# lukehollis/three-mlagents

Hardware: AMD Instinct MI355X
Metric: env_steps_per_sec (higher is better)
Workload: dtype f32; 1 GPU; gridworld, 4096 envs/GPU, full PPO iterations: n_steps=1024, MLP pi/vf 64x64 tanh, n_epochs=10, batch_size=131072/GPU (32 minibatches/epoch), lr=3e-4, gamma=0.99, gae_lambda=0.95, clip=0.2, ent=0.01, vf=0.5, max_grad_norm=0.5; envs_per_gpu=4096, n_steps=1024, batch_size=131072, n_epochs=10, hidden=64, parallelism=single GPU

## Files before the change

include/tma.h:

```cpp
#ifndef TMA_H
#define TMA_H

#include <stdint.h>

#ifdef __cplusplus
extern "C" {
#endif

#define TMA_VERSION 211

enum { TMA_OK = 0, TMA_ERR_INVALID = 1, TMA_ERR_UNKNOWN_TASK = 2, TMA_ERR_HIP = 3 };

enum { TMA_TASK_BASIC = 0, TMA_TASK_GRIDWORLD = 1, TMA_TASK_BALL3D = 2, TMA_TASK_PUSH = 3, TMA_TASK_CRAWLER = 4, TMA_TASK_WALLJUMP = 5, TMA_TASK_BICYCLE = 6, TMA_TASK_BRICKBREAK = 7, TMA_TASK_GLIDER = 8,
       TMA_TASK_ANT = 9,
       TMA_NUM_TASKS = 10 };

enum { TMA_ACT_I32 = 0, TMA_ACT_I64 = 1, TMA_ACT_F32 = 2 };

#define TMA_EP_STRIDE (1u << 20)

int tma_version(void);
const char *tma_last_error(void);

int tma_task_id(const char *name, int *task_out);
// ... 92 lines not shown
                           const tma_ppo_hparams *hp, float *grad, void *workspace, void *stream);
int tma_ppo_epoch_prepare(const tma_rollout *rb, const tma_minibatch *epoch, int64_t batch_size, const tma_policy_dims *d, void *workspace,
                          void *stream);
int tma_ppo_epoch_adv_sums(void *workspace, const tma_policy_dims *d, int64_t batch_size, int64_t total, double *sums, int direction,
                           void *stream);
int tma_ppo_adam_step(float *params, float *grad, float *exp_avg, float *exp_avg_sq, const tma_policy_dims *d, int64_t step, double lr,
                      double beta1, double beta2, double eps, double max_grad_norm, double grad_scale, void *workspace, void *stream);
int tma_ppo_adam_step_local(float *params, float *grad, float *exp_avg, float *exp_avg_sq, const tma_policy_dims *d, int64_t step, double lr,
                            double beta1, double beta2, double eps, double max_grad_norm, void *workspace, void *stream, int64_t last_count);
int tma_ppo_train_epoch_local(float *params, const tma_policy_dims *d, const tma_rollout *rb, uint32_t perm_seed, uint32_t perm_epoch,
                              int64_t batch_size, const tma_ppo_hparams *hp, float *grad, float *exp_avg, float *exp_avg_sq, int64_t first_step,
                              double lr, double beta1, double beta2, double eps, double max_grad_norm, void *workspace, void *stream);
int tma_ppo_train_epochs_local(float *params, const tma_policy_dims *d, const tma_rollout *rb, uint32_t perm_seed, uint32_t perm_epoch0, int n_epochs,
                               int64_t batch_size, const tma_ppo_hparams *hp, float *grad, float *exp_avg, float *exp_avg_sq, int64_t first_step,
                               double lr, double beta1, double beta2, double eps, double max_grad_norm, void *workspace, void *stream);
typedef int (*tma_allreduce_fn)(void *ctx, float *buffer, int64_t count);
int tma_ppo_train_epoch_dp(float *params, const tma_policy_dims *d, const tma_rollout *rb, uint32_t perm_seed, uint32_t perm_epoch,
                           int64_t batch_size, int64_t prepared_batch, int stats_world, const tma_ppo_hparams *hp, float *grad, float *exp_avg,
                           float *exp_avg_sq, int64_t first_step, double lr, double beta1, double beta2, double eps, double max_grad_norm,
                           double grad_scale, tma_allreduce_fn allreduce, void *ctx, void *workspace, void *stream);
typedef struct tma_comm tma_comm;
int tma_comm_available(void);
int tma_comm_unique_id(unsigned char *id_out128);
int tma_comm_create(const unsigned char *id128, int world, int rank, int device, tma_comm **out);
int tma_comm_destroy(tma_comm *comm);
int tma_comm_bind_stream(tma_comm *comm, void *stream);
int tma_comm_allreduce(tma_comm *comm, void *buffer, int64_t count, int dtype, void *stream);
int tma_comm_allreduce_cb(void *ctx, float *buffer, int64_t count);
int tma_comm_timing(tma_comm *comm, int samples);
int tma_comm_pop_timing(tma_comm *comm, float *us_out, int capacity, int *n_out, int64_t *calls_out);
// ... 65 lines not shown
```

three-mlagents_amd/_lib.py:

```python
from __future__ import annotations

import ctypes as C
import os

_HERE = os.path.dirname(os.path.abspath(__file__))
SO_PATH = os.environ.get("TMA_LIB_PATH") or os.path.join(_HERE, "csrc", "libtma_hip.so")

TMA_OK, TMA_ERR_INVALID, TMA_ERR_UNKNOWN_TASK, TMA_ERR_HIP = 0, 1, 2, 3
ACT_I32, ACT_I64, ACT_F32 = 0, 1, 2
EP_STRIDE = 1 << 20
EV_SCRATCH_DOUBLES = 1536

_vp, _i32, _i64, _u32, _f64 = C.c_void_p, C.c_int, C.c_int64, C.c_uint32, C.c_double



class PolicyDims(C.Structure):
    _fields_ = [("obs_dim", _i32), ("hidden", _i32), ("act_dim", _i32), ("continuous", _i32), ("mfma_dtype", _i32), ("device", _i32)]


class Rollout(C.Structure):
    _fields_ = [("obs", _vp), ("actions", _vp), ("log_probs", _vp), ("advantages", _vp), ("returns", _vp), ("T", _i32), ("N", _i64),
                ("packed", _vp)]

# ... 50 lines not shown
    "tma_policy_sync": (_i32, [_vp, _pd, _vp]),
    "tma_policy_act": (_i32, [_vp, _pd, _vp, _i64, _u32, _u32, _u32, _i32, _vp, _vp, _vp, _vp]),
    "tma_policy_act_bootstrap": (_i32, [_vp, _pd, _vp, _i64, _u32, _u32, _u32, _vp, _vp, _vp, _vp, _vp, _f64, _vp, _vp]),
    "tma_policy_evaluate_actions": (_i32, [_vp, _pd, _vp, _vp, _i64, _vp, _vp, _vp, _vp]),
    "tma_policy_values": (_i32, [_vp, _pd, _vp, _i64, _vp, _vp]),
    "tma_policy_bootstrap": (_i32, [_vp, _pd, _vp, _vp, _i64, _f64, _vp, _vp]),
    "tma_ppo_workspace_bytes": (_i64, [_pd]),
    "tma_ppo_packed_floats": (_i64, [_pd, _i32, _i64]),
    "tma_ppo_pack_samples": (_i32, [C.POINTER(Rollout), _pd, _vp, _vp]),
    "tma_ppo_minibatch_grad": (_i32, [_vp, _pd, C.POINTER(Rollout), C.POINTER(Minibatch), C.POINTER(PPOHParams), _vp, _vp, _vp]),
    "tma_debug_time_grad_kernel": (_i32, [_i32]),
    "tma_debug_poison_lds": (_i32, [_u32, _vp]),
    "tma_debug_last_grad_kernel_us": (_i32, [C.POINTER(C.c_float)]),
    "tma_debug_last_dispatch": (_i32, [C.POINTER(_i32), C.POINTER(_i32), C.POINTER(_i32)]),
    "tma_debug_last_rollout_waves": (_i32, []),
    "tma_ppo_epoch_prepare": (_i32, [C.POINTER(Rollout), C.POINTER(Minibatch), _i64, _pd, _vp, _vp]),
    "tma_ppo_epoch_adv_sums": (_i32, [_vp, _pd, _i64, _i64, _vp, _i32, _vp]),
    "tma_ppo_adam_step": (_i32, [_vp, _vp, _vp, _vp, _pd, _i64, _f64, _f64, _f64, _f64, _f64, _f64, _vp, _vp]),
    "tma_ppo_adam_step_local": (_i32, [_vp, _vp, _vp, _vp, _pd, _i64, _f64, _f64, _f64, _f64, _f64, _vp, _vp, _i64]),
    "tma_ppo_permutation": (_i32, [_u32, _u32, _i64, _vp]),
    "tma_ppo_persist_fallbacks": (_i32, [_vp, C.POINTER(_i64), _vp]),
    "tma_ppo_train_epoch_local": (_i32, [_vp, _pd, C.POINTER(Rollout), _u32, _u32, _i64, C.POINTER(PPOHParams), _vp, _vp, _vp, _i64, _f64, _f64, _f64, _f64,
                                         _f64, _vp, _vp]),
    "tma_ppo_train_epochs_local": (_i32, [_vp, _pd, C.POINTER(Rollout), _u32, _u32, _i32, _i64, C.POINTER(PPOHParams), _vp, _vp, _vp, _i64, _f64, _f64, _f64, _f64,
                                          _f64, _vp, _vp]),
    "tma_ppo_train_epoch_dp": (_i32, [_vp, _pd, C.POINTER(Rollout), _u32, _u32, _i64, _i64, _i32, C.POINTER(PPOHParams), _vp, _vp, _vp, _i64, _f64, _f64, _f64,
                                      _f64, _f64, _f64, None, _vp, _vp, _vp]),
    "tma_ppo_pop_stats": (_i32, [_vp, C.POINTER(_f64), _vp]),
    "tma_ppo_stats_staging_bytes": (_i64, []),
    "tma_ppo_stats_enqueue": (_i32, [_vp, _vp, _vp]),
# ... 77 lines not shown
```

three-mlagents_amd/csrc/tma_h64.hip:

```cpp
#include "tma_h64_tile.h"

#include <cstdlib>

namespace tma {


template <int KT, int NT>
__device__ __forceinline__ void bwd_weight_acc(const float *xin, int ldx, int K, const float *dz, int ldz, int N, f32x4 (&accW)[KT][NT],
                                               float (&accb)[NT], int lane) {
    (void)K, (void)N;
    const int r16 = lane & 15, g = lane >> 4;
    float bf[NT][4];
#pragma unroll
    for (int nt = 0; nt < NT; nt++) {
        const int col = nt * 16 + r16;
#pragma unroll
        for (int s = 0; s < 4; s++) bf[nt][s] = dz[(4 * s + g) * ldz + col];
        accb[nt] += (bf[nt][0] + bf[nt][1]) + (bf[nt][2] + bf[nt][3]);
    }
#pragma unroll
    for (int kt = 0; kt < KT; kt++) {
        const int krow = kt * 16 + r16;
        float a[4];
#pragma unroll
// ... 358 lines not shown
        for (int i = 0; i < NO; i++) {
            const int y = o_tid + i * o_thr, x = y < w2_off ? y : y + 4096;
            if (y < n_other) {
                const float gv = (go[i] * f.scale) * coef;
                const float pnew = adam_update_h64(po[i], gv, mo[i], vo[i], f.beta1, f.beta2, inv_bc2, f.eps, f.lr_step);
                image_store_h64(wimg, L.D, n_out, x, pnew);
                if (keep) f.p_nxt[base + x] = pnew, f.m_nxt[base + x] = mo[i], f.v_nxt[base + x] = vo[i];
            }
        }
    }
}

template <bool IS_PI, int DT, bool DIRECT = false, int AT = 0>
__device__ __forceinline__ void grad_h64t_body(const float *__restrict__ params, const PLayout &L, const Rollout &rb, const Minibatch &mb,
                                               const HParams &hp, const double *__restrict__ adv_part, int n_part, float *__restrict__ slab,
                                               double *__restrict__ stat_slot, float *smem, int n_blocks_net, int block_net, const AdamFold &fold) {
#ifdef TMA_H64_TICKS
    const unsigned long long kern_t0 = __builtin_amdgcn_s_memtime();
#endif
    __shared__ float adv_ms[2];
    const int lane = threadIdx.x & 63, wave = threadIdx.x >> 6, wpb = blockDim.x >> 6;
    const int r16 = lane & 15, g = lane >> 4;
    (void)0;
    const int D = DT > 0 ? DT : L.D, A = AT > 0 ? AT : L.A;
    constexpr int KS1C = DT > 0 ? (DT + 3) / 4 : 4;
    const int KS1 = (D + 3) >> 2;
    float *wimg = smem;
    float *slotA = smem + IMG_FLOATS + wave * T_PER_WAVE, *slotB = slotA + 16 * LDT, *dz3t = slotB + 16 * LDT, *Xt = dz3t + 256;
    const float invB = 1.0f / (float)mb.count;
    const int NOUT = IS_PI ? A : 1;
    const int64_t n_tiles = (mb.count + 15) >> 4;
// ... 107 lines not shown
        for (int q = 0; q < 5; q++) red[wave * 5 + q] = stv[q];
    if constexpr (DIRECT) {
        flush_all_t<IS_PI, KS1C, 4>(smem, wave, lane, acc, L, D, NOUT, slab);
    } else {
        flush_all_t<IS_PI, KS1C>(smem, wave, lane, acc, L, D, NOUT, slab);
    }
#ifdef TMA_H64_TICKS
    if (tick_on && lane == 0) g_h64_ticks[IS_PI ? 0 : 1][13] += __builtin_amdgcn_s_memtime() - loop_t1;
#endif
    if (threadIdx.x < 5) {
        double s = 0.0;
        for (int w = 0; w < wpb; w++) s += red[w * 5 + threadIdx.x];
        const int q = IS_PI ? (threadIdx.x == 0 ? 0 : threadIdx.x + 1) : (threadIdx.x == 0 ? 1 : -1);
        if (q >= 0) stat_slot[q] += s;
    }
}

template <int DT, int VER, int AT = 0>
__global__ __launch_bounds__(512, 2) void ppo_grad_h64_kernel(const float *__restrict__ params, PLayout L, Rollout rb, Minibatch mb, HParams hp,
                                                              const double *__restrict__ adv_part, int n_part, float *__restrict__ slabs,
                                                              double *__restrict__ stat_slots, AdamFold fold) {
    extern __shared__ __attribute__((aligned(16))) float smem[];
    const int n_pairs = gridDim.x >> 1, pair = (int)blockIdx.x % n_pairs;
    const bool pi_block = (int)blockIdx.x < n_pairs;
    float *slab = slabs + (int64_t)pair * L.P;
    double *slot = stat_slots + (int64_t)pair * 8;
    if constexpr (VER == 1) {
        if (pi_block) grad_h64_body<true, DT>(params, L, rb, mb, hp, adv_part, n_part, slab, slot, smem, n_pairs, pair);
        else grad_h64_body<false, DT>(params, L, rb, mb, hp, adv_part, n_part, slab, slot, smem, n_pairs, pair);
    } else {
        if (pi_block) grad_h64t_body<true, DT, false, AT>(params, L, rb, mb, hp, adv_part, n_part, slab, slot, smem, n_pairs, pair, fold);
        else grad_h64t_body<false, DT>(params, L, rb, mb, hp, adv_part, n_part, slab, slot, smem, n_pairs, pair, fold);
    }
}

template <int DT>
__global__ __launch_bounds__(256, 1) void ppo_grad_h64_small_kernel(const float *__restrict__ params, PLayout L, Rollout rb, Minibatch mb, HParams hp,
                                                                    const double *__restrict__ adv_part, int n_part, float *__restrict__ slabs,
                                                                    double *__restrict__ stat_slots, AdamFold fold) {
    extern __shared__ __attribute__((aligned(16))) float smem[];
    const int pair = blockIdx.x >> 1, n_pairs = gridDim.x >> 1;
    float *slab = slabs + (int64_t)pair * L.P;
    double *slot = stat_slots + (int64_t)pair * 8;
    if ((blockIdx.x & 1) == 0) grad_h64t_body<true, DT, true>(params, L, rb, mb, hp, adv_part, n_part, slab, slot, smem, n_pairs, pair, fold);
    else grad_h64t_body<false, DT, true>(params, L, rb, mb, hp, adv_part, n_part, slab, slot, smem, n_pairs, pair, fold);
}

}

using namespace tma;

static int grad_h64_smem_bytes(const PLayout &L, int wpb, int ver) {
    const int ldx = ((L.D + 3) & ~3) + 2, ld = L.H + 2;
    const int per_wave = ver == 1 ? 16 * (ldx + 2 * ld + 34) + 16 * 8 : T_PER_WAVE;
    const int tile = (IMG_FLOATS + wpb * per_wave) * 4;
    const int flush = wpb * (L.H * L.H + L.H) * 4;
    return tile > flush ? tile : flush;
}

int tma_launch_grad_h64(const float *params, const PLayout &L, const Rollout &R, const Minibatch &M, const HParams &hpar, const double *adv_part,
                        int n_part, float *slabs, double *slots, int *n_slabs_out, hipStream_t s, const AdamFold *foldp) {
    AdamFold fold{};
    if (foldp) fold = *foldp;
    static const int ver = getenv("TMA_H64_V1") ? 1 : 2;
    if (ver == 1 && foldp && foldp->grad) return TMA_ERR_INVALID;
    static const int stagger = getenv("TMA_H64_STAGGER") ? atoi(getenv("TMA_H64_STAGGER")) : 0;
    static const bool runtime_a = getenv("TMA_H64_RUNTIME_A") != nullptr;
    HParams hps = hpar;
    hps.debug = stagger;
    const int64_t tiles = ceil_div(M.count, 16);
    if (ver == 2 && tiles <= H64_BLOCKS) {
        const int64_t blocks = ceil_div(tiles, 4);
        const int smem = (IMG_FLOATS + 4 * T_PER_WAVE) * 4;
        auto launch_small = [&](auto k) -> int {
            TMA_HIP(hipFuncSetAttribute(reinterpret_cast<const void *>(k), hipFuncAttributeMaxDynamicSharedMemorySize, smem));
            k<<<dim3((unsigned)(2 * blocks)), dim3(256), smem, s>>>(params, L, R, M, hps, adv_part, n_part, slabs, slots, fold);
            return TMA_OK;
        };
        const int rc = L.D == 4 ? launch_small(ppo_grad_h64_small_kernel<4>) : (L.D == 6 ? launch_small(ppo_grad_h64_small_kernel<6>) : launch_small(ppo_grad_h64_small_kernel<0>));
        if (rc) return rc;
        TMA_LAUNCH_CHECK();
        *n_slabs_out = (int)blocks;
        return TMA_OK;
    }
    const int wpb4 = 8, smem4 = grad_h64_smem_bytes(L, wpb4, ver);
    int64_t blocks4 = ceil_div(tiles, wpb4);
    if (blocks4 > H64_BLOCKS) blocks4 = H64_BLOCKS;
    auto launch = [&](auto k) -> int {
        if (smem4 > 64 * 1024) TMA_HIP(hipFuncSetAttribute(reinterpret_cast<const void *>(k), hipFuncAttributeMaxDynamicSharedMemorySize, smem4));
        k<<<dim3((unsigned)(2 * blocks4)), dim3(64 * wpb4), smem4, s>>>(params, L, R, M, hps, adv_part, n_part, slabs, slots, fold);
        return TMA_OK;
    };
    int rc;
    if (ver == 1) rc = L.D == 4 ? launch(ppo_grad_h64_kernel<4, 1>) : (L.D == 6 ? launch(ppo_grad_h64_kernel<6, 1>) : launch(ppo_grad_h64_kernel<0, 1>));
    else if (L.D == 4 && L.A == 5 && !runtime_a) rc = launch(ppo_grad_h64_kernel<4, 2, 5>);
    else rc = L.D == 4 ? launch(ppo_grad_h64_kernel<4, 2>) : (L.D == 6 ? launch(ppo_grad_h64_kernel<6, 2>) : launch(ppo_grad_h64_kernel<0, 2>));
    if (rc) return rc;
    TMA_LAUNCH_CHECK();
    *n_slabs_out = (int)blocks4;
    return TMA_OK;
}

#ifdef TMA_H64_TICKS
extern "C" int tma_debug_h64_ticks(unsigned long long *out32, int reset) {
    TMA_HIP(hipDeviceSynchronize());
    if (out32) TMA_HIP(hipMemcpyFromSymbol(out32, HIP_SYMBOL(g_h64_ticks), sizeof(unsigned long long) * 32));
    if (reset) {
        unsigned long long z[32] = {};
        TMA_HIP(hipMemcpyToSymbol(HIP_SYMBOL(g_h64_ticks), z, sizeof(z)));
    }
    return TMA_OK;
}
#endif
```

three-mlagents_amd/csrc/tma_policy.hip:

```cpp
#include "tma_h64_tile.h"
#include "tma_p2p.h"

#include <cstring>
#include <cmath>
#include <cstdio>
#include <cstdlib>
#include <type_traits>
#include <vector>

namespace tma {


__device__ __forceinline__ void build_image_elem(float *params, const PLayout &L, int img, int e, int W1t, int b1, int W2t, int b2, int W3t, int b3,
                                                 int n_out) {
    const int D = L.D, H = 64;
    float v = 0.0f;
    if (e < IMG_W2F) {
        const int x = e - IMG_W1, k = x >> 6, r16 = (x >> 2) & 15, j = x & 3;
        v = k < D ? params[W1t + k * H + 16 * j + r16] : 0.0f;
    } else if (e < IMG_W3F) {
        const int x = e - IMG_W2F, k = x >> 6, r16 = (x >> 2) & 15, j = x & 3;
        v = params[W2t + k * H + 16 * j + r16];
    } else if (e < IMG_W3B) {
        const int x = e - IMG_W3F, k = x >> 4, col = x & 15;
// ... 219 lines not shown
                            if (entropy_out != nullptr) entropy_out[row] = entsum;
                        }
                        continue;
                    }
                    const float vrow = gfirst_quad(vacc[0][r]);
                    if (r16 == r && row < n) {
                        logp_out[row] = lpsum;
                        values_out[row] = vrow;
                    }
                }
            }
        }
    }
}

constexpr int ADV_BLOCKS = 128;
__global__ __launch_bounds__(256) void adv_partial_kernel(const float *__restrict__ adv, Minibatch mb, int T, int64_t N, double *partials,
                                                          int32_t *__restrict__ offs_out, int64_t batch = 0) {
    __shared__ double s1[4], s2[4];
    if (gridDim.y > 1 || batch > 0) {
        const int64_t k = blockIdx.y, s0 = k * batch;
        const int64_t cnt = (s0 + batch <= mb.count) ? batch : mb.count - s0;
        mb.start += s0, mb.count = cnt;
        partials += 2 * k * gridDim.x;
        if (offs_out) offs_out += s0;
    }
    int nb = (int)((mb.count + 1023) / 1024);
    if (nb > (int)gridDim.x) nb = gridDim.x;
    if ((int)blockIdx.x >= nb) return;
    const int64_t per = (mb.count + nb - 1) / nb;
    const int64_t j0 = (int64_t)blockIdx.x * per, j1 = (j0 + per < mb.count) ? j0 + per : mb.count;
    double a = 0.0, b = 0.0;
    for (int64_t j = j0 + threadIdx.x; j < j1; j += 256) {
        const int64_t off = sample_offset(mb, mb.start + j, T, N);
        if (offs_out) offs_out[j] = (int32_t)off;
        const double x = (double)adv[off];
        a += x;
        b += x * x;
    }
    for (int o = 32; o > 0; o >>= 1) {
        a += __shfl_down(a, o, 64);
        b += __shfl_down(b, o, 64);
    }
    if ((threadIdx.x & 63) == 0) s1[threadIdx.x >> 6] = a, s2[threadIdx.x >> 6] = b;
    __syncthreads();
    if (threadIdx.x == 0) {
        partials[2 * blockIdx.x] = (s1[0] + s1[1]) + (s1[2] + s1[3]);
        partials[2 * blockIdx.x + 1] = (s2[0] + s2[1]) + (s2[2] + s2[3]);
    }
}
__global__ void adv_final_kernel(const double *partials, int n_part, int64_t count, float *ws_adv) {
    double a = 0.0, b = 0.0;
    for (int k = threadIdx.x; k < n_part; k += 64) a += partials[2 * k], b += partials[2 * k + 1];
    for (int o = 32; o > 0; o >>= 1) {
        a += __shfl_down(a, o, 64);
        b += __shfl_down(b, o, 64);
    }
    if (threadIdx.x == 0) {
        const double n = (double)count, mean = a / n;
        double var = n > 1.0 ? (b - n * mean * mean) / (n - 1.0) : 0.0;
        if (var < 0.0) var = 0.0;
        ws_adv[0] = (float)mean;
        ws_adv[1] = (float)sqrt(var);
    }
// ... 2052 lines not shown
    if (n < 1) return fail(TMA_ERR_INVALID, "tma_policy_values: n must be >= 1");
    return launch_fwd<1>(params, d, obs, n, 0, 0, 0, 1, nullptr, values_out, nullptr, nullptr, 0.0f, nullptr, (hipStream_t)stream);
}

int tma_policy_bootstrap(const float *params, const tma_policy_dims *d, const float *terminal_obs, const uint8_t *truncated, int64_t n, double gamma,
                         float *rewards_inout, void *stream) {
    g_disp_fwd = TMA_DISPATCH_NONE;
    int rc = enter(d);
    if (rc) return rc;
    if (!params || !terminal_obs || !truncated || !rewards_inout) return fail(TMA_ERR_INVALID, "tma_policy_bootstrap: null buffer");
    if (n < 1) return fail(TMA_ERR_INVALID, "tma_policy_bootstrap: n must be >= 1");
    return launch_fwd<2>(params, d, terminal_obs, n, 0, 0, 0, 1, nullptr, nullptr, nullptr, truncated, (float)gamma, rewards_inout, (hipStream_t)stream);
}

static int minibatch_grad_impl(const float *params, const tma_policy_dims *d, const tma_rollout *rb, const tma_minibatch *mbi, const tma_ppo_hparams *hp,
                               float *grad, void *workspace, void *stream, const AdamFold *fold, int overwrite, const PeerPush *push = nullptr) {
    g_disp_grad = TMA_DISPATCH_NONE;
    int rc = enter(d);
    if (rc) return rc;
    if (!params || !rb || !mbi || !hp || !grad || !workspace) return fail(TMA_ERR_INVALID, "tma_ppo_minibatch_grad: null argument");
    if (!rb->obs || !rb->actions || !rb->log_probs || !rb->advantages || !rb->returns) return fail(TMA_ERR_INVALID, "rollout view has a null buffer");
    if (rb->T < 1 || rb->N < 1) return fail(TMA_ERR_INVALID, "rollout view: T and N must be >= 1");
    const int64_t total = (int64_t)rb->T * rb->N;
    if (total > 0x7fffffffLL) return fail(TMA_ERR_INVALID, "rollout of %lld samples exceeds the 2^31 minibatch index range", (long long)total);
    if (mbi->count < 1 || mbi->start < 0 || mbi->start + mbi->count > total)
        return fail(TMA_ERR_INVALID, "minibatch [%lld, +%lld) outside the %lld-sample rollout", (long long)mbi->start, (long long)mbi->count, (long long)total);
    hipStream_t s = (hipStream_t)stream;
    const PLayout L = layout_of(d);
    Rollout R{rb->obs, rb->actions, rb->log_probs, rb->advantages, rb->returns, rb->T, rb->N, rec_floats(L) > 0 ? rb->packed : nullptr};
    Minibatch M{mbi->indices, mbi->perm_seed, mbi->perm_epoch, mbi->start, mbi->count, total, nullptr, mbi->count, nullptr, 0};
    const bool prepared = mbi->prepared_batch > 0;
// ... 33 lines not shown
    static const bool force_wide = getenv("TMA_FORCE_WIDE") != nullptr;
    const bool wide_f32 = !L.bf16 && (L.H == 128 || L.H == 192 || L.H == 256) && (tiles >= 8 || force_wide) && grad_wide_smem_bytes(L) <= 160 * 1024;
    if (hpar.normalize_advantage) {
        if (!h64 && !L.bf16 && !wide_f32) {
            adv_final_kernel<<<dim3(1), dim3(64), 0, s>>>(adv_part, nbk, M.stats_n, ws_adv);
            TMA_LAUNCH_CHECK();
        }
    }
    if (h64) {
        g_disp_grad = tiles <= H64_BLOCKS ? TMA_DISPATCH_GRAD_H64_SMALL : TMA_DISPATCH_GRAD_H64;
        float *slabs = reinterpret_cast<float *>(ws + WS_SLABS);
        int blocks4 = 0;
        int lrc;
        {
            GradTimer timer(s);
            lrc = tma_launch_grad_h64(params, L, R, M, hpar, adv_part, nbk, slabs, slots, &blocks4, s, fold);
        }
        if (lrc) return lrc;
        slab_reduce_kernel<<<dim3((unsigned)ceil_div(L.P, 64)), dim3(256), 0, s>>>(slabs, (int)blocks4, L.P, grad, -1, 0, 0, sq_partials(ws, L), overwrite,
                                                                                   push ? *push : PeerPush{});
        TMA_LAUNCH_CHECK();
        return TMA_OK;
    }
    if (fold || overwrite || push) return fail(TMA_ERR_INVALID, "internal: folded optimizer step outside the H = 64 fast path");
    if (L.bf16) {
        g_disp_grad = TMA_DISPATCH_GRAD_BF16;
        if ((int64_t)rb->T * rb->N * L.D >= (int64_t)1 << 31)
            return fail(TMA_ERR_INVALID, "bf16 update: T * N * obs_dim = %lld exceeds 2^31", (long long)((int64_t)rb->T * rb->N * L.D));
        float *slabs = reinterpret_cast<float *>(ws + WS_SLABS);
        int n_pi = 0, n_vf = 0, lrc;
        {
            GradTimer timer(s);
            lrc = tma_launch_grad_wide_bf(params, L, R, M, hpar, ws_adv, slabs, slots, ws, &n_pi, &n_vf, s);
        }
        if (lrc) return lrc;
        slab_reduce_kernel<<<dim3((unsigned)ceil_div(L.P, 64)), dim3(256), 0, s>>>(slabs, n_pi, L.P, grad, n_vf, L.vW1t, L.log_std, sq_partials(ws, L));
        TMA_LAUNCH_CHECK();
        return TMA_OK;
    }
// ... 193 lines not shown
    if (!persist_err) {
        *ran = 1;
        return p256 ? launch_sync(params, L, ps) : TMA_OK;
    }
    TMA_HIP(hipMemsetAsync(ws + WS_PERSIST_ERR, 0, sizeof(int), ps));
    TMA_HIP(hipMemcpyAsync(params, snap, (size_t)L.P * 4, hipMemcpyDeviceToDevice, ps));
    TMA_HIP(hipMemcpyAsync(exp_avg, snap + Pp, (size_t)L.P * 4, hipMemcpyDeviceToDevice, ps));
    TMA_HIP(hipMemcpyAsync(exp_avg_sq, snap + 2 * Pp, (size_t)L.P * 4, hipMemcpyDeviceToDevice, ps));
    TMA_HIP(hipMemcpyAsync(ws + WS_STATS, ws + WS_PERSIST_SNAP, 8 * 8 * 8, hipMemcpyDeviceToDevice, ps));
    rc = launch_sync(params, L, ps);
    if (rc) return rc;
    if (n_epochs == 1) persist_fallback_note(ws, ps);
    return TMA_OK;
}

int tma_ppo_train_epochs_local(float *params, const tma_policy_dims *d, const tma_rollout *rb, uint32_t perm_seed, uint32_t perm_epoch0, int n_epochs,
                               int64_t batch_size, const tma_ppo_hparams *hp, float *grad, float *exp_avg, float *exp_avg_sq, int64_t first_step, double lr,
                               double beta1, double beta2, double eps, double max_grad_norm, void *workspace, void *stream) {
    int rc = enter(d);
    if (rc) return rc;
    if (!params || !rb || !hp || !grad || !exp_avg || !exp_avg_sq || !workspace) return fail(TMA_ERR_INVALID, "tma_ppo_train_epochs_local: null argument");
    if (rb->T < 1 || rb->N < 1 || batch_size < 1 || first_step < 1 || n_epochs < 1)
        return fail(TMA_ERR_INVALID, "tma_ppo_train_epochs_local: T, N, batch_size, first_step and n_epochs must be >= 1");
    const int64_t total = (int64_t)rb->T * rb->N, n_mb = ceil_div(total, batch_size);
    const PLayout L = layout_of(d);
    int e = 0;
    const int per = (int)(total > 0 && OFFS_CAP / total >= 1 ? (OFFS_CAP / total < n_epochs ? OFFS_CAP / total : n_epochs) : 0);
    while (per >= 1 && e < n_epochs) {
        const int n = n_epochs - e < per ? n_epochs - e : per;
        int ran = 0;
        rc = persistent_epochs(params, d, rb, L, perm_seed, perm_epoch0 + (uint32_t)e, n, batch_size, hp, exp_avg, exp_avg_sq, first_step + e * n_mb, lr, beta1, beta2,
                               eps, max_grad_norm, workspace, stream, &ran);
        if (rc) return rc;
        if (!ran) break;
        e += n;
    }
    for (; e < n_epochs; e++) {
        rc = tma_ppo_train_epoch_local(params, d, rb, perm_seed, perm_epoch0 + (uint32_t)e, batch_size, hp, grad, exp_avg, exp_avg_sq, first_step + e * n_mb, lr,
                                       beta1, beta2, eps, max_grad_norm, workspace, stream);
        if (rc) return rc;
    }
    return TMA_OK;
}

int tma_ppo_train_epoch_local(float *params, const tma_policy_dims *d, const tma_rollout *rb, uint32_t perm_seed, uint32_t perm_epoch, int64_t batch_size,
                              const tma_ppo_hparams *hp, float *grad, float *exp_avg, float *exp_avg_sq, int64_t first_step, double lr, double beta1,
                              double beta2, double eps, double max_grad_norm, void *workspace, void *stream) {
    int rc = enter(d);
    if (rc) return rc;
    if (!params || !rb || !hp || !grad || !exp_avg || !exp_avg_sq || !workspace) return fail(TMA_ERR_INVALID, "tma_ppo_train_epoch_local: null argument");
    if (rb->T < 1 || rb->N < 1 || batch_size < 1 || first_step < 1) return fail(TMA_ERR_INVALID, "tma_ppo_train_epoch_local: T, N, batch_size and first_step must be >= 1");
    const int64_t total = (int64_t)rb->T * rb->N;
    const bool prepared = total <= OFFS_CAP && batch_size >= 256;
    const PLayout L = layout_of(d);
    if (prepared) {
        int ran = 0;
        rc = persistent_epochs(params, d, rb, L, perm_seed, perm_epoch, 1, batch_size, hp, exp_avg, exp_avg_sq, first_step, lr, beta1, beta2, eps, max_grad_norm,
                               workspace, stream, &ran);
        if (rc) return rc;
        if (ran) return TMA_OK;
        const tma_minibatch ep{nullptr, perm_seed, perm_epoch, 0, total, 0, 0};
        rc = tma_ppo_epoch_prepare(rb, &ep, batch_size, d, workspace, stream);
        if (rc) return rc;
    }
    int64_t step = first_step;
    const bool no_fold = getenv("TMA_NO_ADAM_FOLD") != nullptr;
    const int64_t tail = total % batch_size;
    if (L.img_pi >= 0 && prepared && (tail == 0 || tail >= 256) && total > batch_size && !no_fold) {
        char *ws = static_cast<char *>(workspace);
        hipStream_t s = (hipStream_t)stream;
        const int64_t Pp = ((int64_t)L.P + 3) & ~(int64_t)3;
        float *alt = reinterpret_cast<float *>(ws + fold_state_offset(L));
        float *bufs[2][3] = {{params, exp_avg, exp_avg_sq}, {alt, alt + Pp, alt + 2 * Pp}};
        int cur = 0;
        const double *sqp = sq_partials(ws, L);
        for (int64_t start = 0; start < total; start += batch_size, step++) {
            const int64_t count = start + batch_size <= total ? batch_size : total - start;
            const tma_minibatch mb{nullptr, perm_seed, perm_epoch, start, count, batch_size, 0};
            AdamFold f{};
            if (start > 0) {
                const double bc1 = 1.0 - pow(beta1, (double)(step - 1)), bc2 = 1.0 - pow(beta2, (double)(step - 1));
                f = AdamFold{grad, sqp, (int)ceil_div(L.P, 64), bufs[cur][0], bufs[cur][1], bufs[cur][2], bufs[cur ^ 1][0], bufs[cur ^ 1][1],
                             bufs[cur ^ 1][2], (float)max_grad_norm, (float)(lr / bc1), (float)beta1, (float)beta2, (float)sqrt(bc2), (float)eps,
                             reinterpret_cast<double *>(ws + WS_NORM_OUT), 1.0f};
            }
            rc = minibatch_grad_impl(params, d, rb, &mb, hp, grad, workspace, stream, start > 0 ? &f : nullptr, start > 0 ? 1 : 0);
            if (rc) return rc;
            if (start > 0) cur ^= 1;
        }
        const double bc1 = 1.0 - pow(beta1, (double)(step - 1)), bc2 = 1.0 - pow(beta2, (double)(step - 1));
        adam_scatter_h64_kernel<<<dim3((unsigned)ceil_div(L.P, 256)), dim3(256), 0, s>>>(
            params, grad, exp_avg, exp_avg_sq, L, sqp, (int)ceil_div(L.P, 64), (float)max_grad_norm, (float)(lr / bc1), (float)beta1, (float)beta2,
            (float)sqrt(bc2), (float)eps, reinterpret_cast<double *>(ws + WS_NORM_OUT), 1.0f, bufs[cur][0], bufs[cur][1], bufs[cur][2]);
        TMA_LAUNCH_CHECK();
        return TMA_OK;
    }
    for (int64_t start = 0; start < total; start += batch_size, step++) {
        const int64_t count = start + batch_size <= total ? batch_size : total - start;
        const tma_minibatch mb{nullptr, perm_seed, perm_epoch, start, count, prepared ? batch_size : 0, 0};
        rc = tma_ppo_minibatch_grad(params, d, rb, &mb, hp, grad, workspace, stream);
        if (rc) return rc;
        rc = tma_ppo_adam_step_local(params, grad, exp_avg, exp_avg_sq, d, step, lr, beta1, beta2, eps, max_grad_norm, workspace, stream, count);
        if (rc) return rc;
    }
    return TMA_OK;
}

int tma_ppo_train_epoch_dp(float *params, const tma_policy_dims *d, const tma_rollout *rb, uint32_t perm_seed, uint32_t perm_epoch, int64_t batch_size,
                           int64_t prepared_batch, int stats_world, const tma_ppo_hparams *hp, float *grad, float *exp_avg, float *exp_avg_sq,
                           int64_t first_step, double lr, double beta1, double beta2, double eps, double max_grad_norm, double grad_scale,
                           tma_allreduce_fn allreduce, void *ctx, void *workspace, void *stream) {
// ... 338 lines not shown
```

three-mlagents_amd/csrc/tma_ppo_types.h:

```cpp
#pragma once
#include "tma_mlp.h"

namespace tma {

constexpr int WS_ADV = 0;
constexpr int WS_NORM_PART = 64;
constexpr int WS_NORM_OUT = 64 + 256 * 8;
constexpr int WS_PERSIST_ERR = 2176;
constexpr int WS_PERSIST_SNAP = 2560;
constexpr int WS_ADV_PART = 4096;
constexpr int WS_STATS = 8192;
constexpr int MAX_GRAD_BLOCKS = 2048;
constexpr int64_t WS_SLABS = WS_STATS + (int64_t)MAX_GRAD_BLOCKS * 8 * 8;
constexpr int H64_BLOCKS = 128;
constexpr int64_t WS_BYTES = WS_SLABS;
constexpr int BF_SLABS = 160;
constexpr int64_t OFFS_CAP = 1 << 22;
constexpr int64_t EPOCH_PART_BYTES = ((OFFS_CAP / 1024) + (OFFS_CAP / 256)) * 16;
constexpr int WIDE_SQ_SLOTS = 8192;

constexpr int64_t DZ1_CAP = 1 << 18;
static inline bool bf_two_pass(const PLayout &L) {
    return L.bf16 && ((L.D > 32 && L.D <= 64) || (L.D > 160 && L.D <= 192) || (L.D > 96 && L.D <= 128 && L.cont && L.H == 256));
}
// ... 9 lines not shown
struct Minibatch {
    const int64_t *indices;
    uint32_t perm_seed, perm_epoch;
    int64_t start, count, total;
    const int32_t *offs;
    int64_t stats_n;
    const double *adv_part;
    int adv_n_part;
};

__device__ __forceinline__ int64_t sample_offset(const Minibatch &mb, int64_t j, int T, int64_t N) {
    const int64_t f = mb.indices ? mb.indices[j] : (int64_t)perm_index(mb.perm_seed, mb.perm_epoch, (uint32_t)j, (uint32_t)mb.total);
    const int64_t i = f / T, t = f - i * T;
    return t * N + i;
}

struct Rollout {
    const float *obs;
    const void *actions;
    const float *log_probs, *advantages, *returns;
    int T;
    int64_t N;
    const float *packed;
};
struct HParams {
    float clip_range, ent_coef, vf_coef;
    int normalize_advantage;
    int debug;
};

// ... 92 lines not shown
            }
        }
        const bool on = valid && r16 == 0;
        st.a += on ? (double)(-fminf(pl1, pl2)) : 0.0;
        st.ent += on ? (double)ent : 0.0;
        st.kl += on ? (double)((ratio - 1.0f) - (lpa - old)) : 0.0;
        st.clip += (on && fabsf(ratio - 1.0f) > hp.clip_range) ? 1.0 : 0.0;
        st.n += on ? 1.0 : 0.0;
    }
}

}

int tma_launch_grad_h64(const float *params, const tma::PLayout &L, const tma::Rollout &R, const tma::Minibatch &M, const tma::HParams &hpar,
                        const double *adv_part, int n_part, float *slabs, double *slots, int *n_slabs_out, hipStream_t s,
                        const tma::AdamFold *fold = nullptr);

bool tma_epoch_h64p_eligible(const tma::PLayout &L, int64_t batch_size, int64_t total);
int tma_launch_epoch_h64p(float *params, const tma::PLayout &L, const tma::Rollout &R, const tma::HParams &hp, const int32_t *offs,
                          const double *adv_part, int adv_stride, int64_t total, int64_t batch_size, float *exp_avg, float *exp_avg_sq,
                          int64_t first_step, double lr, double beta1, double beta2, double eps, double max_grad_norm, char *ws, hipStream_t s);

bool tma_epoch_h256p_eligible(const tma::PLayout &L, int64_t batch_size, int64_t total);
int tma_launch_epoch_h256p(float *params, const tma::PLayout &L, const tma::Rollout &R, const tma::HParams &hp, const int32_t *offs,
                           const double *adv_part, int adv_stride, int64_t total, int64_t batch_size, float *exp_avg, float *exp_avg_sq,
                           int64_t first_step, double lr, double beta1, double beta2, double eps, double max_grad_norm, char *ws, hipStream_t s);

int tma_launch_grad_wide_bf(const float *params, const tma::PLayout &L, const tma::Rollout &R, const tma::Minibatch &M, const tma::HParams &hpar,
                            const float *ws_adv, float *slabs, double *slots, char *ws, int *n_pi_out, int *n_vf_out, hipStream_t s);
int tma_launch_grad_split3(const float *params, const tma::PLayout &L, const tma::Rollout &R, const tma::Minibatch &M, const tma::HParams &hpar, float *slabs,
                           double *slots, int *n_pi_out, int *n_vf_out, hipStream_t s);
// ... 4 lines not shown
```

Before: 131.7 million env-steps/s.

## Fold next minibatch's advantage/offset prep into the H64 value-gradient kernel tail

Instead of running a standalone epoch-prepare pass over all samples, the value-function blocks of the H64 gradient kernel compute the sample offsets and advantage partial sums for the next minibatch at the end of their work. Only the very first minibatch still needs a separate adv_partial launch. This removes per-epoch prepare kernels and overlaps that gather with the gradient kernel's tail. It adds work to the VF blocks, which may lengthen the kernel's critical path. The advantage-sum loop is also unrolled four-wide.

```diff
diff --git a/include/tma.h b/include/tma.h
--- a/include/tma.h
+++ b/include/tma.h
@@ -7,7 +7,7 @@
 extern "C" {
 #endif
 
-#define TMA_VERSION 211
+#define TMA_VERSION 212
 
 enum { TMA_OK = 0, TMA_ERR_INVALID = 1, TMA_ERR_UNKNOWN_TASK = 2, TMA_ERR_HIP = 3 };
 
@@ -130,6 +130,7 @@
 int tma_ppo_train_epochs_local(float *params, const tma_policy_dims *d, const tma_rollout *rb, uint32_t perm_seed, uint32_t perm_epoch0, int n_epochs,
                                int64_t batch_size, const tma_ppo_hparams *hp, float *grad, float *exp_avg, float *exp_avg_sq, int64_t first_step,
                                double lr, double beta1, double beta2, double eps, double max_grad_norm, void *workspace, void *stream);
+int tma_debug_last_prep_fold(int *folded_out, int *standalone_out);
 typedef int (*tma_allreduce_fn)(void *ctx, float *buffer, int64_t count);
 int tma_ppo_train_epoch_dp(float *params, const tma_policy_dims *d, const tma_rollout *rb, uint32_t perm_seed, uint32_t perm_epoch,
                            int64_t batch_size, int64_t prepared_batch, int stats_world, const tma_ppo_hparams *hp, float *grad, float *exp_avg,
diff --git a/three-mlagents_amd/_lib.py b/three-mlagents_amd/_lib.py
--- a/three-mlagents_amd/_lib.py
+++ b/three-mlagents_amd/_lib.py
@@ -88,6 +88,7 @@
     "tma_debug_last_grad_kernel_us": (_i32, [C.POINTER(C.c_float)]),
     "tma_debug_last_dispatch": (_i32, [C.POINTER(_i32), C.POINTER(_i32), C.POINTER(_i32)]),
     "tma_debug_last_rollout_waves": (_i32, []),
+    "tma_debug_last_prep_fold": (_i32, [C.POINTER(_i32), C.POINTER(_i32)]),
     "tma_ppo_epoch_prepare": (_i32, [C.POINTER(Rollout), C.POINTER(Minibatch), _i64, _pd, _vp, _vp]),
     "tma_ppo_epoch_adv_sums": (_i32, [_vp, _pd, _i64, _i64, _vp, _i32, _vp]),
     "tma_ppo_adam_step": (_i32, [_vp, _vp, _vp, _vp, _pd, _i64, _f64, _f64, _f64, _f64, _f64, _f64, _vp, _vp]),
diff --git a/three-mlagents_amd/csrc/tma_h64.hip b/three-mlagents_amd/csrc/tma_h64.hip
--- a/three-mlagents_amd/csrc/tma_h64.hip
+++ b/three-mlagents_amd/csrc/tma_h64.hip
@@ -3,6 +3,10 @@
 #include <cstdlib>
 
 namespace tma {
+
+#ifdef TMA_H64_TICKS
+static __device__ unsigned long long g_h64_tail_ticks;
+#endif
 
 
 template <int KT, int NT>
@@ -396,7 +400,8 @@
 template <bool IS_PI, int DT, bool DIRECT = false, int AT = 0>
 __device__ __forceinline__ void grad_h64t_body(const float *__restrict__ params, const PLayout &L, const Rollout &rb, const Minibatch &mb,
                                                const HParams &hp, const double *__restrict__ adv_part, int n_part, float *__restrict__ slab,
-                                               double *__restrict__ stat_slot, float *smem, int n_blocks_net, int block_net, const AdamFold &fold) {
+                                               double *__restrict__ stat_slot, float *smem, int n_blocks_net, int block_net, const AdamFold &fold,
+                                               const PrepNext &next) {
 #ifdef TMA_H64_TICKS
     const unsigned long long kern_t0 = __builtin_amdgcn_s_memtime();
 #endif
@@ -534,12 +539,28 @@
         const int q = IS_PI ? (threadIdx.x == 0 ? 0 : threadIdx.x + 1) : (threadIdx.x == 0 ? 1 : -1);
         if (q >= 0) stat_slot[q] += s;
     }
+    if constexpr (!IS_PI && !DIRECT) {
+        if (next.count > 0) {
+            __shared__ double prep_s1[4], prep_s2[4];
+            const Minibatch nm{nullptr, next.perm_seed, next.perm_epoch, next.start, next.count, next.total, nullptr, next.count, nullptr, 0};
+            int nb = (int)((next.count + 1023) / 1024);
+            if (nb > ADV_BLOCKS) nb = ADV_BLOCKS;
+            for (int pb = block_net; pb < nb; pb += n_blocks_net) {
+                adv_partial_block(next.adv, nm, next.T, next.N, nb, pb, (int)threadIdx.x, next.partials_out, next.offs_out, next.want_sums != 0, prep_s1,
+                                  prep_s2);
+                __syncthreads();
+            }
+#ifdef TMA_H64_TICKS
+            if (tick_on && lane == 0) g_h64_tail_ticks += __builtin_amdgcn_s_memtime() - loop_t1;
+#endif
+        }
+    }
 }
 
 template <int DT, int VER, int AT = 0>
 __global__ __launch_bounds__(512, 2) void ppo_grad_h64_kernel(const float *__restrict__ params, PLayout L, Rollout rb, Minibatch mb, HParams hp,
                                                               const double *__restrict__ adv_part, int n_part, float *__restrict__ slabs,
-                                                              double *__restrict__ stat_slots, AdamFold fold) {
+                                                              double *__restrict__ stat_slots, AdamFold fold, PrepNext next) {
     extern __shared__ __attribute__((aligned(16))) float smem[];
     const int n_pairs = gridDim.x >> 1, pair = (int)blockIdx.x % n_pairs;
     const bool pi_block = (int)blockIdx.x < n_pairs;
@@ -549,8 +570,8 @@
         if (pi_block) grad_h64_body<true, DT>(params, L, rb, mb, hp, adv_part, n_part, slab, slot, smem, n_pairs, pair);
         else grad_h64_body<false, DT>(params, L, rb, mb, hp, adv_part, n_part, slab, slot, smem, n_pairs, pair);
     } else {
-        if (pi_block) grad_h64t_body<true, DT, false, AT>(params, L, rb, mb, hp, adv_part, n_part, slab, slot, smem, n_pairs, pair, fold);
-        else grad_h64t_body<false, DT>(params, L, rb, mb, hp, adv_part, n_part, slab, slot, smem, n_pairs, pair, fold);
+        if (pi_block) grad_h64t_body<true, DT, false, AT>(params, L, rb, mb, hp, adv_part, n_part, slab, slot, smem, n_pairs, pair, fold, next);
+        else grad_h64t_body<false, DT>(params, L, rb, mb, hp, adv_part, n_part, slab, slot, smem, n_pairs, pair, fold, next);
     }
 }
 
@@ -562,8 +583,8 @@
     const int pair = blockIdx.x >> 1, n_pairs = gridDim.x >> 1;
     float *slab = slabs + (int64_t)pair * L.P;
     double *slot = stat_slots + (int64_t)pair * 8;
-    if ((blockIdx.x & 1) == 0) grad_h64t_body<true, DT, true>(params, L, rb, mb, hp, adv_part, n_part, slab, slot, smem, n_pairs, pair, fold);
-    else grad_h64t_body<false, DT, true>(params, L, rb, mb, hp, adv_part, n_part, slab, slot, smem, n_pairs, pair, fold);
+    if ((blockIdx.x & 1) == 0) grad_h64t_body<true, DT, true>(params, L, rb, mb, hp, adv_part, n_part, slab, slot, smem, n_pairs, pair, fold, PrepNext{});
+    else grad_h64t_body<false, DT, true>(params, L, rb, mb, hp, adv_part, n_part, slab, slot, smem, n_pairs, pair, fold, PrepNext{});
 }
 
 }
@@ -578,12 +599,21 @@
     return tile > flush ? tile : flush;
 }
 
+static int grad_h64_version() {
+    static const int ver = getenv("TMA_H64_V1") ? 1 : 2;
+    return ver;
+}
+bool tma_grad_h64_carries_prep(int64_t count) { return grad_h64_version() == 2 && ceil_div(count, 16) > H64_BLOCKS; }
+
 int tma_launch_grad_h64(const float *params, const PLayout &L, const Rollout &R, const Minibatch &M, const HParams &hpar, const double *adv_part,
-                        int n_part, float *slabs, double *slots, int *n_slabs_out, hipStream_t s, const AdamFold *foldp) {
+                        int n_part, float *slabs, double *slots, int *n_slabs_out, hipStream_t s, const AdamFold *foldp, const PrepNext *nextp) {
     AdamFold fold{};
     if (foldp) fold = *foldp;
-    static const int ver = getenv("TMA_H64_V1") ? 1 : 2;
+    PrepNext next{};
+    if (nextp) next = *nextp;
+    const int ver = grad_h64_version();
     if (ver == 1 && foldp && foldp->grad) return TMA_ERR_INVALID;
+    if (next.count > 0 && !tma_grad_h64_carries_prep(M.count)) return TMA_ERR_INVALID;
     static const int stagger = getenv("TMA_H64_STAGGER") ? atoi(getenv("TMA_H64_STAGGER")) : 0;
     static const bool runtime_a = getenv("TMA_H64_RUNTIME_A") != nullptr;
     HParams hps = hpar;
@@ -608,7 +638,7 @@
     if (blocks4 > H64_BLOCKS) blocks4 = H64_BLOCKS;
     auto launch = [&](auto k) -> int {
         if (smem4 > 64 * 1024) TMA_HIP(hipFuncSetAttribute(reinterpret_cast<const void *>(k), hipFuncAttributeMaxDynamicSharedMemorySize, smem4));
-        k<<<dim3((unsigned)(2 * blocks4)), dim3(64 * wpb4), smem4, s>>>(params, L, R, M, hps, adv_part, n_part, slabs, slots, fold);
+        k<<<dim3((unsigned)(2 * blocks4)), dim3(64 * wpb4), smem4, s>>>(params, L, R, M, hps, adv_part, n_part, slabs, slots, fold, next);
         return TMA_OK;
     };
     int rc;
@@ -622,6 +652,15 @@
 }
 
 #ifdef TMA_H64_TICKS
+extern "C" int tma_debug_h64_tail_ticks(unsigned long long *out, int reset) {
+    TMA_HIP(hipDeviceSynchronize());
+    if (out) TMA_HIP(hipMemcpyFromSymbol(out, HIP_SYMBOL(g_h64_tail_ticks), sizeof(unsigned long long)));
+    if (reset) {
+        unsigned long long z = 0;
+        TMA_HIP(hipMemcpyToSymbol(HIP_SYMBOL(g_h64_tail_ticks), &z, sizeof(z)));
+    }
+    return TMA_OK;
+}
 extern "C" int tma_debug_h64_ticks(unsigned long long *out32, int reset) {
     TMA_HIP(hipDeviceSynchronize());
     if (out32) TMA_HIP(hipMemcpyFromSymbol(out32, HIP_SYMBOL(g_h64_ticks), sizeof(unsigned long long) * 32));
diff --git a/three-mlagents_amd/csrc/tma_policy.hip b/three-mlagents_amd/csrc/tma_policy.hip
--- a/three-mlagents_amd/csrc/tma_policy.hip
+++ b/three-mlagents_amd/csrc/tma_policy.hip
@@ -257,7 +257,6 @@
     }
 }
 
-constexpr int ADV_BLOCKS = 128;
 __global__ __launch_bounds__(256) void adv_partial_kernel(const float *__restrict__ adv, Minibatch mb, int T, int64_t N, double *partials,
                                                           int32_t *__restrict__ offs_out, int64_t batch = 0) {
     __shared__ double s1[4], s2[4];
@@ -271,26 +270,7 @@
     int nb = (int)((mb.count + 1023) / 1024);
     if (nb > (int)gridDim.x) nb = gridDim.x;
     if ((int)blockIdx.x >= nb) return;
-    const int64_t per = (mb.count + nb - 1) / nb;
-    const int64_t j0 = (int64_t)blockIdx.x * per, j1 = (j0 + per < mb.count) ? j0 + per : mb.count;
-    double a = 0.0, b = 0.0;
-    for (int64_t j = j0 + threadIdx.x; j < j1; j += 256) {
-        const int64_t off = sample_offset(mb, mb.start + j, T, N);
-        if (offs_out) offs_out[j] = (int32_t)off;
-        const double x = (double)adv[off];
-        a += x;
-        b += x * x;
-    }
-    for (int o = 32; o > 0; o >>= 1) {
-        a += __shfl_down(a, o, 64);
-        b += __shfl_down(b, o, 64);
-    }
-    if ((threadIdx.x & 63) == 0) s1[threadIdx.x >> 6] = a, s2[threadIdx.x >> 6] = b;
-    __syncthreads();
-    if (threadIdx.x == 0) {
-        partials[2 * blockIdx.x] = (s1[0] + s1[1]) + (s1[2] + s1[3]);
-        partials[2 * blockIdx.x + 1] = (s2[0] + s2[1]) + (s2[2] + s2[3]);
-    }
+    adv_partial_block(adv, mb, T, N, nb, (int)blockIdx.x, (int)threadIdx.x, partials, offs_out, true, s1, s2);
 }
 __global__ void adv_final_kernel(const double *partials, int n_part, int64_t count, float *ws_adv) {
     double a = 0.0, b = 0.0;
@@ -2373,7 +2353,8 @@
 }
 
 static int minibatch_grad_impl(const float *params, const tma_policy_dims *d, const tma_rollout *rb, const tma_minibatch *mbi, const tma_ppo_hparams *hp,
-                               float *grad, void *workspace, void *stream, const AdamFold *fold, int overwrite, const PeerPush *push = nullptr) {
+                               float *grad, void *workspace, void *stream, const AdamFold *fold, int overwrite, const PeerPush *push = nullptr,
+                               const PrepNext *next = nullptr ) {
     g_disp_grad = TMA_DISPATCH_NONE;
     int rc = enter(d);
     if (rc) return rc;
@@ -2437,7 +2418,7 @@
         int lrc;
         {
             GradTimer timer(s);
-            lrc = tma_launch_grad_h64(params, L, R, M, hpar, adv_part, nbk, slabs, slots, &blocks4, s, fold);
+            lrc = tma_launch_grad_h64(params, L, R, M, hpar, adv_part, nbk, slabs, slots, &blocks4, s, fold, next);
         }
         if (lrc) return lrc;
         slab_reduce_kernel<<<dim3((unsigned)ceil_div(L.P, 64)), dim3(256), 0, s>>>(slabs, (int)blocks4, L.P, grad, -1, 0, 0, sq_partials(ws, L), overwrite,
@@ -2445,7 +2426,7 @@
         TMA_LAUNCH_CHECK();
         return TMA_OK;
     }
-    if (fold || overwrite || push) return fail(TMA_ERR_INVALID, "internal: folded optimizer step outside the H = 64 fast path");
+    if (fold || overwrite || push || next) return fail(TMA_ERR_INVALID, "internal: folded optimizer step outside the H = 64 fast path");
     if (L.bf16) {
         g_disp_grad = TMA_DISPATCH_GRAD_BF16;
         if ((int64_t)rb->T * rb->N * L.D >= (int64_t)1 << 31)
@@ -2669,6 +2650,96 @@
     return TMA_OK;
 }
 
+static thread_local int g_prep_folded = 0, g_prep_standalone = 0;
+
+static bool h64_fold_eligible(const PLayout &L, int64_t total, int64_t batch_size) {
+    const bool no_fold = getenv("TMA_NO_ADAM_FOLD") != nullptr;
+    const int64_t tail = total % batch_size;
+    return L.img_pi >= 0 && total <= OFFS_CAP && batch_size >= 256 && (tail == 0 || tail >= 256) && total > batch_size && !no_fold;
+}
+
+static int h64_fold_epochs(float *params, const tma_policy_dims *d, const tma_rollout *rb, const PLayout &L, uint32_t perm_seed, uint32_t perm_epoch0, int n_epochs,
+                           int64_t batch_size, const tma_ppo_hparams *hp, float *grad, float *exp_avg, float *exp_avg_sq, int64_t first_step, double lr,
+                           double beta1, double beta2, double eps, double max_grad_norm, void *workspace, void *stream) {
+    if (!rb->obs || !rb->actions || !rb->log_probs || !rb->advantages || !rb->returns) return fail(TMA_ERR_INVALID, "rollout view has a null buffer");
+    const int64_t total = (int64_t)rb->T * rb->N, n_mb = ceil_div(total, batch_size);
+    char *ws = static_cast<char *>(workspace);
+    hipStream_t s = (hipStream_t)stream;
+    const int64_t Pp = ((int64_t)L.P + 3) & ~(int64_t)3;
+    float *alt = reinterpret_cast<float *>(ws + fold_state_offset(L));
+    float *bufs[2][3] = {{params, exp_avg, exp_avg_sq}, {alt, alt + Pp, alt + 2 * Pp}};
+    int cur = 0;
+    const double *sqp = sq_partials(ws, L);
+    const bool chain = getenv("TMA_NO_PREP_FOLD") == nullptr && tma_grad_h64_carries_prep(batch_size);
+    const int64_t offs_base = WS_SLABS + (int64_t)slab_cap(L) * L.P * 4;
+    int32_t *offs_all = reinterpret_cast<int32_t *>(ws + offs_base);
+    double *part_all = reinterpret_cast<double *>(ws + offs_base + OFFS_CAP * 4);
+    int stride = (int)ceil_div(batch_size, 1024);
+    if (stride > ADV_BLOCKS) stride = ADV_BLOCKS;
+    auto prep_of = [&](int e, int64_t k) {
+        const int64_t start = k * batch_size, count = start + batch_size <= total ? batch_size : total - start;
+        return PrepNext{rb->advantages, offs_all + start, part_all + 2 * k * stride, perm_seed, perm_epoch0 + (uint32_t)e, start, count, total, rb->N, rb->T,
+                        hp->normalize_advantage ? 1 : 0};
+    };
+    bool ready = false;
+    int64_t step = first_step;
+    int rc;
+    for (int e = 0; e < n_epochs; e++) {
+        if (!chain) {
+            const tma_minibatch ep{nullptr, perm_seed, perm_epoch0 + (uint32_t)e, 0, total, 0, 0};
+            rc = tma_ppo_epoch_prepare(rb, &ep, batch_size, d, workspace, stream);
+            if (rc) return rc;
+            g_prep_standalone++;
+        }
+        for (int64_t k = 0; k < n_mb; k++, step++) {
+            const PrepNext me = prep_of(e, k);
+            if (chain && !ready) {
+                const Minibatch M{nullptr, me.perm_seed, me.perm_epoch, me.start, me.count, total, nullptr, me.count, nullptr, 0};
+                int nbk = (int)ceil_div(me.count, 1024);
+                if (nbk > ADV_BLOCKS) nbk = ADV_BLOCKS;
+                adv_partial_kernel<<<dim3(nbk), dim3(256), 0, s>>>(rb->advantages, M, rb->T, rb->N, me.partials_out, me.offs_out);
+                TMA_LAUNCH_CHECK();
+                g_prep_standalone++;
+            }
+            ready = false;
+            PrepNext nx{};
+            if (chain && (k + 1 < n_mb || e + 1 < n_epochs)) {
+                nx = k + 1 < n_mb ? prep_of(e, k + 1) : prep_of(e + 1, 0);
+                ready = tma_grad_h64_carries_prep(me.count) && tma_grad_h64_carries_prep(nx.count);
+                if (ready) g_prep_folded++;
+            }
+            const tma_minibatch mb{nullptr, perm_seed, me.perm_epoch, me.start, me.count, batch_size, 0};
+            AdamFold f{};
+            if (k > 0) {
+                const double bc1 = 1.0 - pow(beta1, (double)(step - 1)), bc2 = 1.0 - pow(beta2, (double)(step - 1));
+                f = AdamFold{grad, sqp, (int)ceil_div(L.P, 64), bufs[cur][0], bufs[cur][1], bufs[cur][2], bufs[cur ^ 1][0], bufs[cur ^ 1][1],
+                             bufs[cur ^ 1][2], (float)max_grad_norm, (float)(lr / bc1), (float)beta1, (float)beta2, (float)sqrt(bc2), (float)eps,
+                             reinterpret_cast<double *>(ws + WS_NORM_OUT), 1.0f};
+            }
+            rc = minibatch_grad_impl(params, d, rb, &mb, hp, grad, workspace, stream, k > 0 ? &f : nullptr, k > 0 ? 1 : 0, nullptr, ready ? &nx : nullptr);
+            if (rc) return rc;
+            if (k > 0) cur ^= 1;
+        }
+        const double bc1 = 1.0 - pow(beta1, (double)(step - 1)), bc2 = 1.0 - pow(beta2, (double)(step - 1));
+        adam_scatter_h64_kernel<<<dim3((unsigned)ceil_div(L.P, 256)), dim3(256), 0, s>>>(
+            params, grad, exp_avg, exp_avg_sq, L, sqp, (int)ceil_div(L.P, 64), (float)max_grad_norm, (float)(lr / bc1), (float)beta1, (float)beta2,
+            (float)sqrt(bc2), (float)eps, reinterpret_cast<double *>(ws + WS_NORM_OUT), 1.0f, bufs[cur][0], bufs[cur][1], bufs[cur][2]);
+        TMA_LAUNCH_CHECK();
+        cur = 0;
+    }
+    return TMA_OK;
+}
+
+int tma_debug_last_prep_fold(int *folded_out, int *standalone_out) {
+    if (folded_out) *folded_out = g_prep_folded;
+    if (standalone_out) *standalone_out = g_prep_standalone;
+    return TMA_OK;
+}
+
+static int train_epoch_local_impl(float *params, const tma_policy_dims *d, const tma_rollout *rb, uint32_t perm_seed, uint32_t perm_epoch, int64_t batch_size,
+                                  const tma_ppo_hparams *hp, float *grad, float *exp_avg, float *exp_avg_sq, int64_t first_step, double lr, double beta1,
+                                  double beta2, double eps, double max_grad_norm, void *workspace, void *stream);
+
 int tma_ppo_train_epochs_local(float *params, const tma_policy_dims *d, const tma_rollout *rb, uint32_t perm_seed, uint32_t perm_epoch0, int n_epochs,
                                int64_t batch_size, const tma_ppo_hparams *hp, float *grad, float *exp_avg, float *exp_avg_sq, int64_t first_step, double lr,
                                double beta1, double beta2, double eps, double max_grad_norm, void *workspace, void *stream) {
@@ -2679,6 +2750,7 @@
         return fail(TMA_ERR_INVALID, "tma_ppo_train_epochs_local: T, N, batch_size, first_step and n_epochs must be >= 1");
     const int64_t total = (int64_t)rb->T * rb->N, n_mb = ceil_div(total, batch_size);
     const PLayout L = layout_of(d);
+    g_prep_folded = g_prep_standalone = 0;
     int e = 0;
     const int per = (int)(total > 0 && OFFS_CAP / total >= 1 ? (OFFS_CAP / total < n_epochs ? OFFS_CAP / total : n_epochs) : 0);
     while (per >= 1 && e < n_epochs) {
@@ -2690,8 +2762,11 @@
         if (!ran) break;
         e += n;
     }
+    if (e < n_epochs && h64_fold_eligible(L, total, batch_size) && tma_grad_h64_carries_prep(batch_size))
+        return h64_fold_epochs(params, d, rb, L, perm_seed, perm_epoch0 + (uint32_t)e, n_epochs - e, batch_size, hp, grad, exp_avg, exp_avg_sq, first_step + e * n_mb, lr,
+                               beta1, beta2, eps, max_grad_norm, workspace, stream);
     for (; e < n_epochs; e++) {
-        rc = tma_ppo_train_epoch_local(params, d, rb, perm_seed, perm_epoch0 + (uint32_t)e, batch_size, hp, grad, exp_avg, exp_avg_sq, first_step + e * n_mb, lr,
+        rc = train_epoch_local_impl(params, d, rb, perm_seed, perm_epoch0 + (uint32_t)e, batch_size, hp, grad, exp_avg, exp_avg_sq, first_step + e * n_mb, lr,
                                        beta1, beta2, eps, max_grad_norm, workspace, stream);
         if (rc) return rc;
     }
@@ -2701,6 +2776,14 @@
 int tma_ppo_train_epoch_local(float *params, const tma_policy_dims *d, const tma_rollout *rb, uint32_t perm_seed, uint32_t perm_epoch, int64_t batch_size,
                               const tma_ppo_hparams *hp, float *grad, float *exp_avg, float *exp_avg_sq, int64_t first_step, double lr, double beta1,
                               double beta2, double eps, double max_grad_norm, void *workspace, void *stream) {
+    g_prep_folded = g_prep_standalone = 0;
+    return train_epoch_local_impl(params, d, rb, perm_seed, perm_epoch, batch_size, hp, grad, exp_avg, exp_avg_sq, first_step, lr, beta1, beta2, eps, max_grad_norm,
+                                  workspace, stream);
+}
+
+static int train_epoch_local_impl(float *params, const tma_policy_dims *d, const tma_rollout *rb, uint32_t perm_seed, uint32_t perm_epoch, int64_t batch_size,
+                                  const tma_ppo_hparams *hp, float *grad, float *exp_avg, float *exp_avg_sq, int64_t first_step, double lr, double beta1,
+                                  double beta2, double eps, double max_grad_norm, void *workspace, void *stream) {
     int rc = enter(d);
     if (rc) return rc;
     if (!params || !rb || !hp || !grad || !exp_avg || !exp_avg_sq || !workspace) return fail(TMA_ERR_INVALID, "tma_ppo_train_epoch_local: null argument");
@@ -2714,42 +2797,15 @@
                                workspace, stream, &ran);
         if (rc) return rc;
         if (ran) return TMA_OK;
+        if (h64_fold_eligible(L, total, batch_size))
+            return h64_fold_epochs(params, d, rb, L, perm_seed, perm_epoch, 1, batch_size, hp, grad, exp_avg, exp_avg_sq, first_step, lr, beta1, beta2, eps,
+                                   max_grad_norm, workspace, stream);
         const tma_minibatch ep{nullptr, perm_seed, perm_epoch, 0, total, 0, 0};
         rc = tma_ppo_epoch_prepare(rb, &ep, batch_size, d, workspace, stream);
         if (rc) return rc;
+        g_prep_standalone++;
     }
     int64_t step = first_step;
-    const bool no_fold = getenv("TMA_NO_ADAM_FOLD") != nullptr;
-    const int64_t tail = total % batch_size;
-    if (L.img_pi >= 0 && prepared && (tail == 0 || tail >= 256) && total > batch_size && !no_fold) {
-        char *ws = static_cast<char *>(workspace);
-        hipStream_t s = (hipStream_t)stream;
-        const int64_t Pp = ((int64_t)L.P + 3) & ~(int64_t)3;
-        float *alt = reinterpret_cast<float *>(ws + fold_state_offset(L));
-        float *bufs[2][3] = {{params, exp_avg, exp_avg_sq}, {alt, alt + Pp, alt + 2 * Pp}};
-        int cur = 0;
-        const double *sqp = sq_partials(ws, L);
-        for (int64_t start = 0; start < total; start += batch_size, step++) {
-            const int64_t count = start + batch_size <= total ? batch_size : total - start;
-            const tma_minibatch mb{nullptr, perm_seed, perm_epoch, start, count, batch_size, 0};
-            AdamFold f{};
-            if (start > 0) {
-                const double bc1 = 1.0 - pow(beta1, (double)(step - 1)), bc2 = 1.0 - pow(beta2, (double)(step - 1));
-                f = AdamFold{grad, sqp, (int)ceil_div(L.P, 64), bufs[cur][0], bufs[cur][1], bufs[cur][2], bufs[cur ^ 1][0], bufs[cur ^ 1][1],
-                             bufs[cur ^ 1][2], (float)max_grad_norm, (float)(lr / bc1), (float)beta1, (float)beta2, (float)sqrt(bc2), (float)eps,
-                             reinterpret_cast<double *>(ws + WS_NORM_OUT), 1.0f};
-            }
-            rc = minibatch_grad_impl(params, d, rb, &mb, hp, grad, workspace, stream, start > 0 ? &f : nullptr, start > 0 ? 1 : 0);
-            if (rc) return rc;
-            if (start > 0) cur ^= 1;
-        }
-        const double bc1 = 1.0 - pow(beta1, (double)(step - 1)), bc2 = 1.0 - pow(beta2, (double)(step - 1));
-        adam_scatter_h64_kernel<<<dim3((unsigned)ceil_div(L.P, 256)), dim3(256), 0, s>>>(
-            params, grad, exp_avg, exp_avg_sq, L, sqp, (int)ceil_div(L.P, 64), (float)max_grad_norm, (float)(lr / bc1), (float)beta1, (float)beta2,
-            (float)sqrt(bc2), (float)eps, reinterpret_cast<double *>(ws + WS_NORM_OUT), 1.0f, bufs[cur][0], bufs[cur][1], bufs[cur][2]);
-        TMA_LAUNCH_CHECK();
-        return TMA_OK;
-    }
     for (int64_t start = 0; start < total; start += batch_size, step++) {
         const int64_t count = start + batch_size <= total ? batch_size : total - start;
         const tma_minibatch mb{nullptr, perm_seed, perm_epoch, start, count, prepared ? batch_size : 0, 0};
diff --git a/three-mlagents_amd/csrc/tma_ppo_types.h b/three-mlagents_amd/csrc/tma_ppo_types.h
--- a/three-mlagents_amd/csrc/tma_ppo_types.h
+++ b/three-mlagents_amd/csrc/tma_ppo_types.h
@@ -47,6 +47,66 @@
     const int64_t i = f / T, t = f - i * T;
     return t * N + i;
 }
+
+constexpr int ADV_BLOCKS = 128;
+__device__ __forceinline__ void adv_partial_block(const float *__restrict__ adv, const Minibatch &mb, int T, int64_t N, int nb, int pb, int tid,
+                                                  double *__restrict__ partials, int32_t *__restrict__ offs_out, bool want_sums, double *s1,
+                                                  double *s2) {
+    const int64_t per = (mb.count + nb - 1) / nb;
+    const int64_t j0 = (int64_t)pb * per, j1 = (j0 + per < mb.count) ? j0 + per : mb.count;
+    if (tid < 256) {
+        double a = 0.0, b = 0.0;
+        for (int64_t j = j0 + tid; j < j1; j += 4 * 256) {
+            int64_t off[4];
+            float x[4];
+#pragma unroll
+            for (int q = 0; q < 4; q++) {
+                const int64_t jq = j + 256 * q;
+                off[q] = 0;
+                if (jq < j1) {
+                    off[q] = sample_offset(mb, mb.start + jq, T, N);
+                    if (offs_out) offs_out[jq] = (int32_t)off[q];
+                }
+            }
+            if (want_sums) {
+#pragma unroll
+                for (int q = 0; q < 4; q++) x[q] = adv[off[q]];
+#pragma unroll
+                for (int q = 0; q < 4; q++) {
+                    if (j + 256 * q < j1) {
+                        const double xd = (double)x[q];
+                        a += xd;
+                        b += xd * xd;
+                    }
+                }
+            }
+        }
+        if (want_sums) {
+            for (int o = 32; o > 0; o >>= 1) {
+                a += __shfl_down(a, o, 64);
+                b += __shfl_down(b, o, 64);
+            }
+            if ((tid & 63) == 0) s1[tid >> 6] = a, s2[tid >> 6] = b;
+        }
+    }
+    if (!want_sums) return;
+    __syncthreads();
+    if (tid == 0) {
+        partials[2 * pb] = (s1[0] + s1[1]) + (s1[2] + s1[3]);
+        partials[2 * pb + 1] = (s2[0] + s2[1]) + (s2[2] + s2[3]);
+    }
+}
+
+struct PrepNext {
+    const float *adv;
+    int32_t *offs_out;
+    double *partials_out;
+    uint32_t perm_seed, perm_epoch;
+    int64_t start, count, total;
+    int64_t N;
+    int T;
+    int want_sums;
+};
 
 struct Rollout {
     const float *obs;
@@ -169,7 +229,8 @@
 
 int tma_launch_grad_h64(const float *params, const tma::PLayout &L, const tma::Rollout &R, const tma::Minibatch &M, const tma::HParams &hpar,
                         const double *adv_part, int n_part, float *slabs, double *slots, int *n_slabs_out, hipStream_t s,
-                        const tma::AdamFold *fold = nullptr);
+                        const tma::AdamFold *fold = nullptr, const tma::PrepNext *next = nullptr);
+bool tma_grad_h64_carries_prep(int64_t count);
 
 bool tma_epoch_h64p_eligible(const tma::PLayout &L, int64_t batch_size, int64_t total);
 int tma_launch_epoch_h64p(float *params, const tma::PLayout &L, const tma::Rollout &R, const tma::HParams &hp, const int32_t *offs,
```

Measured after the change: 134.2 million env-steps/s, median of 6. 1.9% higher.
